# AbrahamSanders/realtime-codec-agent

Hardware: AMD Instinct MI355X
Metric: batch-encode audio-hours/hour (+ xRT and p50 frame-step latency of 1 duplex stream in `duplex`) (higher is better)
Workload: dtype f32; 1 GPU; batch MagiCodec-style encode, 16 kHz stereo, 0.1 s chunks / 2.0 s context, 256 windows per step (BASELINE configs[1]); codebook=131072x16

## Files before the change

realtime_codec_agent_amd/csrc/rca_codec.hip:

```cpp
#include <stdarg.h>

#include <algorithm>
#include <array>
#include <cmath>
#include <map>
#include <type_traits>

#include "rca_common.h"

namespace rca {
thread_local char g_err[512] = {0};
}
using namespace rca;

typedef float f32x16 __attribute__((ext_vector_type(16)));

#define RCA_LAT_MAX_FRAMES 64
#define RCA_LDS_BUDGET (152 * 1024)

typedef float f32x4 __attribute__((ext_vector_type(4)));

struct RowSrc {
    const float* base;
    int C;
    long chan_stride;
    long win_stride;
    int T;
    const long* row_off = nullptr;
    long span = 0;
    __device__ __forceinline__ long off(long b) const {
        return row_off ? row_off[b] : (b % C) * chan_stride + (b / C) * win_stride;
    }
};

__device__ __forceinline__ float lrelu(float v, float slope) { return v >= 0.0f ? v : v * slope; }

template <int KS>
__global__ __launch_bounds__(256) void conv_in_kernel(RowSrc src, const float* __restrict__ w,
                                                      const float* __restrict__ bias, float* __restrict__ y,
                                                      int B, int Cout, int Lout) {
    const long idx = (long)blockIdx.x * blockDim.x + threadIdx.x;
    if (idx >= (long)B * Lout) return;
    const int b = (int)(idx / Lout);
    const int t = (int)(idx - (long)b * Lout);
    const float* xr = src.base + src.off(b);
    constexpr int padL = KS / 2;
    float xv[KS];
#pragma unroll
    for (int kk = 0; kk < KS; ++kk) {
        const int i = t + kk - padL;
        xv[kk] = (i >= 0 && i < src.T) ? xr[i] : 0.0f;
    }
    float* yo = y + (long)b * Cout * Lout + t;
    for (int co = 0; co < Cout; ++co) {
        float acc = bias[co];
#pragma unroll
        for (int kk = 0; kk < KS; ++kk) {
            const int i = t + kk - padL;
            if (i >= 0 && i < src.T) acc = __builtin_fmaf(w[co * KS + kk], xv[kk], acc);
        }
        yo[(long)co * Lout] = acc;
    }
}

__global__ __launch_bounds__(256) void conv1d_chain_kernel(const float* __restrict__ x, const float* __restrict__ w,
                                                           const float* __restrict__ bias, float* __restrict__ y,
                                                           int B, int Cin, int Lin, int Cout, int Lout, int k, int s,
                                                           int pre, float slope, int clamp_out) {
    const long idx = (long)blockIdx.x * blockDim.x + threadIdx.x;
    if (idx >= (long)B * Cout * Lout) return;
    const int t = (int)(idx % Lout);
    const long r = idx / Lout;
    const int co = (int)(r % Cout);
    const int b = (int)(r / Cout);
    const int padL = (k - s + 1) / 2;
    const float* xb = x + (long)b * Cin * Lin;
    const float* wr = w + (long)co * Cin * k;
    float acc = bias[co];
    const int i0 = t * s - padL;
    for (int ci = 0; ci < Cin; ++ci) {
        const float* xr = xb + (long)ci * Lin;
        for (int kk = 0; kk < k; ++kk) {
            const int i = i0 + kk;
            if (i >= 0 && i < Lin) {
                float v = xr[i];
                if (pre) v = lrelu(v, slope);
                acc = __builtin_fmaf(wr[ci * k + kk], v, acc);
            }
        }
    }
    if (clamp_out) acc = acc > 1.0f ? 1.0f : (acc < -1.0f ? -1.0f : acc);
// ... 74 lines not shown
};
struct TrInfo {
    int s, padL, Lout, n_co;
};
template <int KS, int S, int TR>
struct ConvBOff {
    static constexpr int padL = (KS - S + 1) / 2;
    static constexpr int q_of(int kp, int half) {
        const int kl = 2 * kp + half, kk = kl % KS;
        const int d = TR ? -kk : kk - padL;
        return (d >= 0) ? d / S : -((-d + S - 1) / S);
    }
    static constexpr int off(int kp, int half, int U) {
        const int kl = 2 * kp + half, ci = kl / KS, kk = kl % KS;
        const int d = TR ? -kk : kk - padL;
        const int q = q_of(kp, half);
        return (ci * S + (d - q * S)) * U + 1 + q;
    }
    static constexpr int delta(int kp, int U) { return off(kp, 1, U) - off(kp, 0, U); }
    static constexpr int distinct(int k, int KPC, int U) {
        int found[4] = {0, 0, 0, 0};
        int n = 0;
        for (int kp = 0; kp < KPC; ++kp) {
            const int d = delta(kp, U);
            bool seen = false;
            for (int i = 0; i < n; ++i) seen = seen || found[i] == d;
            if (!seen && n < 4) found[n++] = d;
        }
        return found[k < n ? k : n - 1];
    }
    static constexpr int count(int KPC, int U) {
        int found[8] = {0, 0, 0, 0, 0, 0, 0, 0};
        int n = 0;
        for (int kp = 0; kp < KPC; ++kp) {
            const int d = delta(kp, U);
            bool seen = false;
            for (int i = 0; i < n; ++i) seen = seen || found[i] == d;
            if (!seen && n < 8) found[n++] = d;
        }
        return n;
    }
};

#ifndef RCA_CONV_WPB
#define RCA_CONV_WPB 1
#endif
#ifndef RCA_CONV_OCC
#define RCA_CONV_OCC 2
#endif
#ifndef RCA_CONV_PIPE
#define RCA_CONV_PIPE 1
#endif
#ifndef RCA_CONV_PRIO
#define RCA_CONV_PRIO 1
#endif
#ifndef RCA_CONV_ABUF
#define RCA_CONV_ABUF 1
#endif
#ifndef RCA_CONV_EPRIO
#define RCA_CONV_EPRIO 1
#endif
#ifdef RCA_ABL_NOBREAD
#define RCA_ABL_BREAD(x) (slope)
#else
#define RCA_ABL_BREAD(x) (x)
#endif
typedef __bf16 conv_bf16x8 __attribute__((ext_vector_type(8)));
typedef __bf16 conv_bf16x2 __attribute__((ext_vector_type(2)));
__device__ __forceinline__ unsigned conv_pack_bf16x2(float a, float b) {
    const conv_bf16x2 v = {(__bf16)a, (__bf16)b};
    return __builtin_bit_cast(unsigned, v);
}
template <int BF>
__device__ __forceinline__ void conv_split8(const float (&w)[8], uint4& hi, uint4& lo) {
    unsigned ph[4], pl[4];
#pragma unroll
    for (int j = 0; j < 4; ++j) {
        ph[j] = conv_pack_bf16x2(w[2 * j], w[2 * j + 1]);
        pl[j] = BF == 3 ? conv_pack_bf16x2(w[2 * j] - __uint_as_float(ph[j] << 16), w[2 * j + 1] - __uint_as_float(ph[j] & 0xffff0000u)) : 0u;
    }
    hi = make_uint4(ph[0], ph[1], ph[2], ph[3]);
    lo = make_uint4(pl[0], pl[1], pl[2], pl[3]);
}
template <int KS, int S, int CIC, int WM, int WN, int FUSE, int TR, int BF = 0, int FULLC = 0>
__global__ __launch_bounds__(64 * RCA_CONV_WPB, (((KS == 8 && CIC == 2) || (KS == 16 && CIC == 1)) && WM * WN < 8) ? 3 : RCA_CONV_OCC) void conv1d_mfma_kernel(const float* __restrict__ x, const float* __restrict__ wp,
                                                          const float* __restrict__ bias, float* __restrict__ y,
                                                          int Cin, int Lin, int Cout, int Lout, long Ncols, int nchunks,
                                                          int pre, float slope, FuseIn fin, TrInfo tr) {
    constexpr int MT = WM * 32;
    constexpr int NW = WN * 32;
    constexpr int U = ConvLds<S>::stride(NW);
    constexpr int KPC = CIC * KS / 2;
    constexpr int QPC = KPC / 4;
    constexpr int E = (NW + 2) * S;
    constexpr int PW = (S % 2 == 0 && !TR) ? 2 : 1;
    constexpr int RE = (E + 64 * PW - 1) / (64 * PW);
    constexpr int padL = (KS - S + 1) / 2;
    constexpr int BUF = CIC * S * U + 4;
    static_assert((CIC * KS) % 8 == 0, "chunk must hold whole weight quads");

    extern __shared__ __attribute__((aligned(16))) float xs_all[];
#ifdef RCA_CONV_TIMELINE
    long* const tl_buf = rca_prof_buf;
#endif
    RCA_TL_STAMP(tl0);

    const int lane = threadIdx.x & 63;
    const int half = lane >> 5;
    const int wave = __builtin_amdgcn_readfirstlane(threadIdx.x >> 6);
    float* xs = xs_all + wave * 2 * BUF;
    const int n_co_real = (Cout + MT - 1) / MT;
    const int n_co = TR ? n_co_real * tr.s : n_co_real;
    const long wg = blockIdx.x;
    const int xcd = (int)(wg & 7);
    const long seq = wg >> 3;
    const int co_tile_x = __builtin_amdgcn_readfirstlane((int)(seq % n_co));
    const int phase = TR ? co_tile_x / n_co_real : 0;
    const int co_tile = TR ? co_tile_x % n_co_real : co_tile_x;
    const long col_tile = (seq / n_co) * 8 + xcd;
    const long n0 = (col_tile * RCA_CONV_WPB + wave) * NW;
    const int co0 = co_tile * MT;
    if (n0 >= Ncols) return;
    const long n_base = n0 > 0 ? n0 - 1 : 0;
    const int b_base = __builtin_amdgcn_readfirstlane((int)((unsigned)n_base / (unsigned)Lout));
    const int t_base = (int)(n_base - (long)b_base * Lout);
    const int lead = n0 > 0 ? 0 : 1;
    const long left = Ncols - n_base;
    const int ncol_left = left > NW + 2 ? NW + 2 : (int)left;
    auto rel_bt = [&](int dn, int& bb, int& tt) {
        int dt = dn + t_base;
        bb = 0;
        if (Lout >= NW + 3) {
            if (dt >= Lout) { dt -= Lout; bb = 1; }
        } else {
            bb = dt / Lout;
            dt -= bb * Lout;
        }
        tt = dt;
    };

    constexpr unsigned OOB = 0x80000000u;
    const rca_rsrc_t rs_x = rca_make_rsrc(FUSE ? fin.src.base : x + (long)b_base * Cin * Lin, 0x7FFFFFFF);
    const rca_rsrc_t rs_none = rca_make_rsrc(FUSE ? fin.src.base : x, 0);
    unsigned s_boff[RE];
    int s_loff[RE];
    bool s_ok[FUSE ? RE : 1];
    float pc[FUSE ? RE : 1][6 + PW];
    rca_rsrc_t rs_pcm = rs_none;
    unsigned prow[2] = {0u, 0u};
    if (FUSE) {
        long o0, o1;
        if (fin.src.row_off) {
            const long nrows = (Ncols + Lout - 1) / Lout;
            o0 = fin.src.row_off[b_base];
            o1 = fin.src.row_off[b_base + 1 < nrows ? b_base + 1 : b_base];
        } else {
            const int C = fin.src.C;
            const int c0 = b_base % C, w0 = b_base / C;
            const int c1 = c0 + 1 == C ? 0 : c0 + 1, w1 = c0 + 1 == C ? w0 + 1 : w0;
            o0 = (long)c0 * fin.src.chan_stride + (long)w0 * fin.src.win_stride;
            o1 = (long)c1 * fin.src.chan_stride + (long)w1 * fin.src.win_stride;
        }
        const long om = o0 < o1 ? o0 : o1;
        rs_pcm = rca_make_rsrc(fin.src.base + om, 0x7FFFFFFF);
        prow[0] = (unsigned)(o0 - om);
        prow[1] = (unsigned)(o1 - om);
    }
#pragma unroll
    for (int r = 0; r < RE; ++r) {
        const int e = PW * (lane + 64 * r);
        const int slot = e / S, p = e - slot * S;
        const int dn = slot - lead;
        bool ok = e < E && dn >= 0 && dn < ncol_left;
        int bb, t;
        rel_bt(ok ? dn : 0, bb, t);
        if (TR && t >= Lin) ok = false;
        s_loff[r] = e < E ? p * U + slot : (U > NW + 2 ? U - 1 : -1);
        s_boff[r] = ok ? ((unsigned)bb * (unsigned)(Cin * Lin) + (unsigned)(t * S + p)) * 4u : OOB;
        if (FUSE) {
            s_ok[r] = ok;
            const int i = t * S + p;
            const unsigned ro = bb ? prow[1] : prow[0];
#pragma unroll
            for (int kk = 0; kk < 6 + PW; ++kk) {
                const int j = i + kk - 3;
                const unsigned off = (ok && j >= 0 && j < fin.src.T) ? (ro + (unsigned)j) * 4u : OOB;
                pc[r][kk] = rca_buffer_load_f32(rs_pcm, (int)off, 0, 0);
            }
        }
    }
    float sreg[CIC][RE][PW];
    auto stage_load = [&](int c) {
#pragma unroll
        for (int cl = 0; cl < CIC; ++cl) {
            const int ci = c * CIC + cl;
            if (FUSE) {
                const int cc = ci < Cin ? ci : 0;
                const float* wr = fin.w_in + cc * 7;
                const float bi = fin.b_in[cc];
#pragma unroll
                for (int r = 0; r < RE; ++r)
#pragma unroll
                    for (int j = 0; j < PW; ++j) {
// ... 281 lines not shown
        }
        RCA_TL_STAMP(td);
        RCA_TL_MIN(tl_load, tb, tc); RCA_TL_ADD(tl_mfma, tb, tc); RCA_TL_ADD(tl_write, tc, td);
        if (c + 1 >= nchunks) break;
        const int c2 = min(c + 2, lastc);
        stage_load(c2);
        __builtin_amdgcn_sched_barrier(0);
        __builtin_amdgcn_s_setprio(RCA_CONV_EPRIO);
        if constexpr (BF != 0) compute_b(1, c2, edge_tag);
        else if constexpr (PIPE) compute_p(1, c2, edge_tag);
        else compute_t(1, c2, edge_tag);
        __builtin_amdgcn_s_setprio(RCA_CONV_PRIO ? 3 : 2);
        __builtin_amdgcn_sched_barrier(0);
        stage_write_t(0, act_tag);
        __builtin_amdgcn_wave_barrier();
        if constexpr (PIPE) {
            read_head(0);
            __builtin_amdgcn_sched_barrier(0);
        }
    }
    };
    if (pre & 1) {
        if (edges) chunk_loop(std::true_type{}, std::true_type{});
        else chunk_loop(std::false_type{}, std::true_type{});
    } else {
        if (edges) chunk_loop(std::true_type{}, std::false_type{});
        else chunk_loop(std::false_type{}, std::false_type{});
    }

    if (RCA_CONV_EPRIO) __builtin_amdgcn_s_setprio(0);
    RCA_TL_STAMP(tl2);
    const long orow = TR ? tr.Lout : Lout;
    const bool full_rows = co0 + MT <= Cout;
    float* const yw = y + ((long)b_base * Cout + co0) * orow;
#pragma unroll
    for (int wn = 0; wn < WN; ++wn) {
        const int dn = 1 - lead + wn * 32 + (lane & 31);
        if (dn >= ncol_left) continue;
        int bb, t;
        rel_bt(dn, bb, t);
        int ocol = t;
        if (TR) {
            ocol = tr.s * t - tr.padL + phase;
            if (ocol < 0 || ocol >= (int)orow) continue;
        }
        const unsigned voff = ((unsigned)bb * (unsigned)(Cout * (int)orow) + (unsigned)ocol + (unsigned)(4 * half) * (unsigned)orow) * 4u;
        if (pre & 2) {
#pragma unroll
            for (int wm = 0; wm < WM; ++wm)
#pragma unroll
                for (int r = 0; r < 16; ++r) acc[wm][wn][r] = fmaxf(acc[wm][wn][r], acc[wm][wn][r] * slope);
        }
        if (full_rows) {
#pragma unroll
            for (int wm = 0; wm < WM; ++wm)
#pragma unroll
                for (int r = 0; r < 16; ++r) {
                    const int cu = wm * 32 + (r & 3) + 8 * (r >> 2);
                    char* const yr = reinterpret_cast<char*>(yw + (long)cu * orow);
                    *reinterpret_cast<float*>(yr + voff) = acc[wm][wn][r];
                }
        } else {
#pragma unroll
            for (int wm = 0; wm < WM; ++wm)
#pragma unroll
                for (int r = 0; r < 16; ++r) {
                    const int cu = wm * 32 + (r & 3) + 8 * (r >> 2);
                    char* const yr = reinterpret_cast<char*>(yw + (long)cu * orow);
                    if (co0 + cu + 4 * half < Cout) *reinterpret_cast<float*>(yr + voff) = acc[wm][wn][r];
                }
        }
    }
#ifdef RCA_CONV_TIMELINE
    if (tl_buf && lane == 0) {
        const long tl3 = (long)wall_clock64();
        const unsigned hw = __builtin_amdgcn_s_getreg((31 << 11) | (0 << 6) | 4);
        const unsigned xcc = __builtin_amdgcn_s_getreg((3 << 11) | (0 << 6) | 20);
        constexpr int region = KS == 4 ? 0 : KS == 8 ? 1 : KS == 10 ? 2 : KS == 16 ? 3 : KS == 3 ? 4 : 5;
        long* o = tl_buf + ((long)region * 65536 + ((blockIdx.x * RCA_CONV_WPB + wave) & 0xFFFF)) * 8;
        o[6] = tl_load | (tl_mfma << 32);
        o[7] = tl_write | ((long)nchunks << 32);
        o[0] = tl0; o[1] = tl1; o[2] = tl2; o[3] = tl3;
        o[4] = (long)hw | ((long)xcc << 32);
        o[5] = (long)KS | ((long)S << 8) | ((long)WM << 16) | ((long)wave << 24) | ((long)blockIdx.x << 32);
    }
#endif
}

template <int NWN, bool PRE>
__global__ __launch_bounds__(64, 2) void conv_first_mfma_kernel(const float* __restrict__ wp, const float* __restrict__ bias,
                                                               float* __restrict__ y, int Cout, int Lout, long Ncols, int post, float slope,
                                                               FuseIn fin) {
    constexpr int NW = NWN * 32;
    constexpr int E = (NW + 2) * 2;
    constexpr int NBLK = 2 * NWN + 1;
    constexpr int RS = 136;
    constexpr int ZERO = 128;
    constexpr int CIN = 32, KQ = CIN / 2;
    extern __shared__ __attribute__((aligned(16))) float ring[];
#ifdef RCA_CONV_TIMELINE
    long* const tl_buf = rca_prof_buf;
#endif
    RCA_TL_STAMP(tl0);
    const int lane = threadIdx.x & 63;
    const int half = lane >> 5, jl = lane & 31;
    const int n_co = Cout / 64;
    const long wg = blockIdx.x;
    const int xcd = (int)(wg & 7);
    const long seq = wg >> 3;
    const int co_tile = __builtin_amdgcn_readfirstlane((int)(seq % n_co));
    const long n0 = ((seq / n_co) * 8 + xcd) * NW;
    const int co0 = co_tile * 64;
    if (n0 >= Ncols) return;
    const long n_base = n0 > 0 ? n0 - 1 : 0;
    const int b_base = __builtin_amdgcn_readfirstlane((int)((unsigned)n_base / (unsigned)Lout));
    const int t_base = (int)(n_base - (long)b_base * Lout);
    const int lead = n0 > 0 ? 0 : 1;
    const long left = Ncols - n_base;
    const int ncol_left = left > NW + 2 ? NW + 2 : (int)left;
    auto rel_bt = [&](int dn, int& bb, int& tt) {
        int dt = dn + t_base;
        bb = dt >= Lout ? 1 : 0;
        tt = bb ? dt - Lout : dt;
    };

    const int ch_in = jl;
    float a_in[4];
#pragma unroll
    for (int m = 0; m < 4; ++m) a_in[m] = (2 * m + half < 7) ? fin.w_in[ch_in * 7 + 2 * m + half] : -0.0f;
    f32x16 b_in;
#pragma unroll
    for (int r = 0; r < 16; ++r) b_in[r] = fin.b_in[(r & 3) + 8 * (r >> 2) + 4 * half];
    long o0, o1;
    if (fin.src.row_off) {
        const long nrows = (Ncols + Lout - 1) / Lout;
        o0 = fin.src.row_off[b_base];
        o1 = fin.src.row_off[b_base + 1 < nrows ? b_base + 1 : b_base];
    } else {
        const int C = fin.src.C;
        const int c0 = b_base % C, w0 = b_base / C;
        const int c1 = c0 + 1 == C ? 0 : c0 + 1, w1 = c0 + 1 == C ? w0 + 1 : w0;
        o0 = (long)c0 * fin.src.chan_stride + (long)w0 * fin.src.win_stride;
        o1 = (long)c1 * fin.src.chan_stride + (long)w1 * fin.src.win_stride;
    }
    const long om = o0 < o1 ? o0 : o1;
    const rca_rsrc_t rs_pcm = rca_make_rsrc(fin.src.base + om, 0x7FFFFFFF);
    const unsigned prow0 = (unsigned)(o0 - om), prow1 = (unsigned)(o1 - om);
    constexpr unsigned OOB = 0x80000000u;
    auto pcm_load = [&](int bk, float (&pb)[4]) __attribute__((always_inline)) {
        const int e = 32 * bk + jl;
        const int dn = (e >> 1) - lead;
        const bool ok = e < E && dn >= 0 && dn < ncol_left;
        int bb, t;
        rel_bt(ok ? dn : 0, bb, t);
        const int i = 2 * t + (e & 1) - 3 + half;
        const unsigned ro = bb ? prow1 : prow0;
#pragma unroll
        for (int m = 0; m < 4; ++m) {
            const int j = i + 2 * m;
            const unsigned off = (ok && 2 * m + half < 7 && j >= 0 && j < fin.src.T) ? (ro + (unsigned)j) * 4u : OOB;
            pb[m] = rca_buffer_load_f32(rs_pcm, (int)off, 0, 0);
        }
    };
    auto cin_mfma = [&](int m, const float (&pb)[4], f32x16& d) __attribute__((always_inline)) {
        d = __builtin_amdgcn_mfma_f32_32x32x2f32(a_in[m], pb[m], m == 0 ? b_in : d, 0, 0, 0);
    };
    const int w_lane = 4 * half * RS + jl;
    auto cin_write = [&](int bk, f32x16& d, int r0, int r1) __attribute__((always_inline)) {
#pragma unroll
// ... 1441 lines not shown
                v.push_back(L);
                return fail(RCA_ERR_HIP, "bias pad alloc");
            }
        }
        if (pack && !tr && mfma_supported(k, s)) {
            const rca_tensor_t* t = find_tensor(ts, nt, name + ".weight");
            if ((rc = pack_weights((const float*)t->data, L)) != RCA_OK) { v.push_back(L); return rc; }
        }
        if (tr && k == 2 * s) {
            const rca_tensor_t* t = find_tensor(ts, nt, name + ".weight");
            if ((rc = pack_weights_tr((const float*)t->data, L)) != RCA_OK) { v.push_back(L); return rc; }
        }
        v.push_back(L);
        return RCA_OK;
    };
    if ((rc = add(h->enc, "enc.conv_in", 1, cfg->channels[0], cfg->k_in, 1, 0, 0, false)) != RCA_OK) return bail(rc);
    for (int i = 0; i < n; ++i) {
        const int s = cfg->strides[i];
        if ((rc = add(h->enc, "enc.down." + std::to_string(i), cfg->channels[i], cfg->channels[i + 1], 2 * s, s, 1, 0, true)) != RCA_OK)
            return bail(rc);
    }
    if ((rc = add(h->enc, "enc.conv_out", cfg->channels[n], cfg->latent_dim, cfg->k_latent, 1, 1, 0, true)) != RCA_OK) return bail(rc);
    if ((rc = add(h->dec, "dec.conv_in", cfg->codebook_dim, cfg->channels[n], cfg->k_latent, 1, 0, 0, true)) != RCA_OK) return bail(rc);
    for (int i = 0; i < n; ++i) {
        const int s = cfg->strides[n - 1 - i];
        if ((rc = add(h->dec, "dec.up." + std::to_string(i), cfg->channels[n - i], cfg->channels[n - 1 - i], 2 * s, s, 1, 1, false)) != RCA_OK)
            return bail(rc);
    }
    if ((rc = add(h->dec, "dec.conv_out", cfg->channels[0], 1, cfg->k_in, 1, 1, 0, false)) != RCA_OK) return bail(rc);

    const int J = cfg->codebook_dim, N = cfg->codebook_size, R = cfg->codebook_raw_dim, D = cfg->latent_dim;
    if ((rc = upload(ts, nt, "quantizer.in_proj.weight", (long)J * D, &h->q_in_w)) != RCA_OK) return bail(rc);
    if ((rc = upload(ts, nt, "quantizer.in_proj.bias", J, &h->q_in_b)) != RCA_OK) return bail(rc);
    float *raw = nullptr, *pw = nullptr, *pb = nullptr;
    auto free3 = [&]() { for (float* p : {raw, pw, pb}) if (p) (void)hipFree(p); };
    if ((rc = upload(ts, nt, "quantizer.codebook.weight", (long)N * R, &raw)) != RCA_OK) { free3(); return bail(rc); }
    if ((rc = upload(ts, nt, "quantizer.codebook_proj.weight", (long)J * R, &pw)) != RCA_OK) { free3(); return bail(rc); }
    if ((rc = upload(ts, nt, "quantizer.codebook_proj.bias", J, &pb)) != RCA_OK) { free3(); return bail(rc); }
    if (hipMalloc((void**)&h->cb, (size_t)N * J * 4) != hipSuccess || hipMalloc((void**)&h->hc, (size_t)N * 4) != hipSuccess ||
        hipMalloc((void**)&h->cbp, (size_t)N * J * 4) != hipSuccess || hipMalloc((void**)&h->err_flag, 4) != hipSuccess) {
        free3();
        return bail(fail(RCA_ERR_HIP, "codebook alloc"));
    }
    (void)hipMemsetAsync(h->err_flag, 0, 4, h->stream);
#ifdef RCA_CONV_TIMELINE
    if (getenv("RCA_CONV_TIMELINE_OUT")) {
        long* b = nullptr;
        (void)hipMalloc((void**)&b, (size_t)(6 << 16) * 8 * 8);
        (void)hipMemset(b, 0, (size_t)(6 << 16) * 8 * 8);
        (void)hipMemcpyToSymbol(HIP_SYMBOL(rca_prof_buf), &b, 8);
    }
#endif
    codebook_proj_kernel<<<cdiv((long)N * J, 256), 256, 0, h->stream>>>(raw, pw, pb, h->cb, N, R, J);
    codebook_norm_pack_kernel<<<cdiv(N, 256), 256, 0, h->stream>>>(h->cb, h->hc, h->cbp, N, J);
    hipError_t e = hipStreamSynchronize(h->stream);
    free3();
    if (e != hipSuccess) return bail(fail(RCA_ERR_HIP, "codebook init: %s", hipGetErrorString(e)));
    *out = h;
    return RCA_OK;
}

extern "C" int rca_codec_hop(const rca_codec_t* h, int32_t* hop) {
    if (!h || !hop) return fail(RCA_ERR_ARG, "null");
    *hop = h->hop;
    return RCA_OK;
}
extern "C" int rca_codec_num_frames(const rca_codec_t* h, int32_t T, int32_t* F) {
    if (!h || !F || T < 0) return fail(RCA_ERR_ARG, "bad argument");
    *F = (T + h->hop - 1) / h->hop;
    return RCA_OK;
}
extern "C" int rca_codec_set_variant(rca_codec_t* h, int32_t v) {
    if (!h || v < 0 || v > 2) return fail(RCA_ERR_ARG, "variant must be 0, 1 or 2");
    h->variant = v;
    return RCA_OK;
}
extern "C" int rca_codec_sync(rca_codec_t* h) {
    if (!h) return fail(RCA_ERR_ARG, "null");
    RCA_HIP(hipSetDevice(h->device));
    RCA_HIP(hipStreamSynchronize(h->stream));
    return RCA_OK;
}

template <int KS, int S, int CIC, int WM, int WN, int FUSE, int TR, int BF = 0>
static void launch_conv_cfg(const ConvLayer& L, const float* wp, int nchunks, const float* x, float* y, int Lin, int Lc, long Ncols,
                            float slope, const FuseIn& fin, const TrInfo& tr, hipStream_t st, int act) {
    constexpr int NT = RCA_CONV_WPB * WN * 32, MT = WM * 32;
    constexpr int lds = RCA_CONV_WPB * 2 * (CIC * S * ConvLds<S>::stride(WN * 32) + 4) * 4;
    static_assert(lds <= 65536, "LDS budget");
    const long col_tiles = (cdiv(Ncols, NT) + 7) / 8 * 8;
    dim3 grid((unsigned)(col_tiles * cdiv(L.cout, MT) * (TR ? tr.s : 1)));
    if constexpr (!FUSE && !TR && BF == 0) {
        if (L.cin % CIC == 0 && nchunks * CIC == L.cin) {
            conv1d_mfma_kernel<KS, S, CIC, WM, WN, 0, 0, 0, 1><<<grid, 64 * RCA_CONV_WPB, lds, st>>>(x, wp, L.bp, y, L.cin, Lin, L.cout, Lc, Ncols, nchunks, act, slope, fin, tr);
            return;
        }
    }
    conv1d_mfma_kernel<KS, S, CIC, WM, WN, FUSE, TR, BF><<<grid, 64 * RCA_CONV_WPB, lds, st>>>(x, wp, L.bp, y, L.cin, Lin, L.cout, Lc, Ncols, nchunks, act, slope, fin, tr);
}

template <int KS, int S, int CIC>
static int launch_conv_mfma(const ConvLayer& L, const float* x, float* y, int B, int Lin, int Lout, float slope, hipStream_t st,
                            const FuseIn* fuse = nullptr, int act = -1, int bf = 0) {
    if (act < 0) act = L.pre;
    const long Ncols = (long)B * Lout;
    if (bf) {
        const FuseIn none_b{};
        const TrInfo notr_b{};
        const bool big = (long)cdiv(Ncols, 64) * cdiv(L.cout, 64) >= 2048;
#define RCA_BF_LAUNCH(FU, BFM) do { \
            if (big) launch_conv_cfg<KS, S, CIC, 2, 2, FU, 0, BFM>(L, L.wp, L.nchunks, x, y, Lin, Lout, Ncols, slope, FU ? *fuse : none_b, notr_b, st, act); \
            else launch_conv_cfg<KS, S, CIC, 1, 1, FU, 0, BFM>(L, L.wp, L.nchunks, x, y, Lin, Lout, Ncols, slope, FU ? *fuse : none_b, notr_b, st, act); } while (0)
        if constexpr (KS == 4 || KS == 8 || KS == 16) {
            if (fuse) { if (bf == 3) RCA_BF_LAUNCH(1, 3); else RCA_BF_LAUNCH(1, 1); RCA_LAUNCH_CHECK(); return RCA_OK; }
        }
        if (fuse) return fail(RCA_ERR_ARG, "internal: fused first layer of this shape has no bf16 instantiation");
        if (bf == 3) RCA_BF_LAUNCH(0, 3); else RCA_BF_LAUNCH(0, 1);
#undef RCA_BF_LAUNCH
        RCA_LAUNCH_CHECK();
        return RCA_OK;
    }
    const long waves_big = (long)cdiv(Ncols, 64) * cdiv(L.cout, 64);
#ifdef RCA_CONV_FORCE_MID
    constexpr long BIG_MIN = 1L << 40, MID_MIN = 2048;
#else
    constexpr long BIG_MIN = 8192, MID_MIN = 2048;
#endif
    const FuseIn none{};
    const TrInfo notr{};
    if (fuse) {
        static const bool wide = []() { const char* e = getenv("RCA_FUSE_WIDE"); return !(e && e[0] == '0'); }();
        if constexpr (KS == 4 && S == 2) {
            const char* mi = getenv("RCA_FUSE_MFMA_IN");
            constexpr int NWN = 4;
            if (!(mi && mi[0] == '0') && wide && waves_big >= BIG_MIN && Lout >= NWN * 32 + 3 && L.cin == 32 && L.cout % 64 == 0) {
                const long col_tiles = (cdiv(Ncols, NWN * 32) + 7) / 8 * 8;
                const dim3 grid((unsigned)(col_tiles * (L.cout / 64)));
                constexpr int lds = 32 * 136 * 4;
                if (act & 1) conv_first_mfma_kernel<NWN, true><<<grid, 64, lds, st>>>(L.wp, L.bp, y, L.cout, Lout, Ncols, act & 2, slope, *fuse);
                else conv_first_mfma_kernel<NWN, false><<<grid, 64, lds, st>>>(L.wp, L.bp, y, L.cout, Lout, Ncols, act & 2, slope, *fuse);
                RCA_LAUNCH_CHECK();
                return RCA_OK;
            }
            if (wide && waves_big >= BIG_MIN && Lout >= 131 && L.cin % 2 == 0) {
                launch_conv_cfg<4, 2, 2, 2, 4, 1, 0>(L, L.wp, L.cin / 2, x, y, Lin, Lout, Ncols, slope, *fuse, notr, st, act);
                RCA_LAUNCH_CHECK();
                return RCA_OK;
            }
        }
        if (waves_big >= BIG_MIN) launch_conv_cfg<KS, S, CIC, 2, 2, 1, 0>(L, L.wp, L.nchunks, x, y, Lin, Lout, Ncols, slope, *fuse, notr, st, act);
        else launch_conv_cfg<KS, S, CIC, 1, 1, 1, 0>(L, L.wp, L.nchunks, x, y, Lin, Lout, Ncols, slope, *fuse, notr, st, act);
    } else {
        if (waves_big >= BIG_MIN) launch_conv_cfg<KS, S, CIC, 2, 2, 0, 0>(L, L.wp, L.nchunks, x, y, Lin, Lout, Ncols, slope, none, notr, st, act);
        else if (waves_big >= MID_MIN) launch_conv_cfg<KS, S, CIC, 1, 2, 0, 0>(L, L.wp, L.nchunks, x, y, Lin, Lout, Ncols, slope, none, notr, st, act);
        else if (KS == 3 && L.cout >= 64 && waves_big >= 1024) launch_conv_cfg<KS, S, CIC, (KS == 3 ? 2 : 1), 1, 0, 0>(L, L.wp, L.nchunks, x, y, Lin, Lout, Ncols, slope, none, notr, st, act);
        else launch_conv_cfg<KS, S, CIC, 1, 1, 0, 0>(L, L.wp, L.nchunks, x, y, Lin, Lout, Ncols, slope, none, notr, st, act);
    }
    RCA_LAUNCH_CHECK();
    return RCA_OK;
}

static int launch_convtr_mfma(const ConvLayer& L, const float* x, float* y, int B, int Lin, float slope, hipStream_t st) {
    const int Lc = Lin + 1;
    const long Ncols = (long)B * Lc;
    const FuseIn none{};
    const TrInfo tr{L.s, (L.k - L.s + 1) / 2, Lin * L.s, L.cout_pad / 32};
    const long waves_big = (long)cdiv(Ncols, 64) * cdiv(L.cout, 64) * L.s;
    if (L.cout > 32 && waves_big >= 2048) launch_conv_cfg<2, 1, 16, 2, 2, 0, 1>(L, L.wp_tr, L.nchunks_tr, x, y, Lin, Lc, Ncols, slope, none, tr, st, L.pre);
    else launch_conv_cfg<2, 1, 16, 1, 1, 0, 1>(L, L.wp_tr, L.nchunks_tr, x, y, Lin, Lc, Ncols, slope, none, tr, st, L.pre);
    RCA_LAUNCH_CHECK();
    return RCA_OK;
}

template <int KS, int S, int CIC, int FUSE>
static void launch_conv_ws(const ConvLayer& L, const float* x, float* y, int Lin, int Lout, long Ncols, float slope, const FuseIn& fin,
                           hipStream_t st) {
    constexpr int KPC = CIC * KS / 2, QPC = KPC / 4;
    constexpr int lds = (2 * (2 * QPC * 64 * 4) + 4 * 2 * (CIC * S * ConvLds<S>::stride(64) + 4)) * 4;
    static_assert(lds <= 160 * 1024, "LDS budget");
    auto kern = conv1d_ws_kernel<KS, S, CIC, FUSE>;
    static bool attr_done = false;
    if (!attr_done) { (void)hipFuncSetAttribute((const void*)kern, hipFuncAttributeMaxDynamicSharedMemorySize, lds); attr_done = true; }
    const long col_tiles = (cdiv(Ncols, 256) + 7) / 8 * 8;
    dim3 grid((unsigned)(col_tiles * cdiv(L.cout, 64)));
    kern<<<grid, 512, lds, st>>>(x, L.wp2, L.b, y, L.cin, Lin, L.cout, Lout, Ncols, L.nchunks2, L.pre, slope, fin);
}
static bool try_conv_ws(const ConvLayer& L, const float* x, float* y, int B, int Lin, int Lout, float slope, hipStream_t st, const FuseIn* fuse) {
    const long Ncols = (long)B * Lout;
    if (!L.wp2 || (long)cdiv(Ncols, 64) * cdiv(L.cout, 64) < 1024) return false;
    const FuseIn none{};
    if (L.k == 4 && L.s == 2) { if (fuse) launch_conv_ws<4, 2, 16, 1>(L, x, y, Lin, Lout, Ncols, slope, *fuse, st); else launch_conv_ws<4, 2, 16, 0>(L, x, y, Lin, Lout, Ncols, slope, none, st); }
    else if (L.k == 8 && L.s == 4 && !fuse) launch_conv_ws<8, 4, 8, 0>(L, x, y, Lin, Lout, Ncols, slope, none, st);
    else if (L.k == 16 && L.s == 8 && !fuse) launch_conv_ws<16, 8, 4, 0>(L, x, y, Lin, Lout, Ncols, slope, none, st);
    else if (L.k == 10 && L.s == 5 && !fuse) launch_conv_ws<10, 5, 8, 0>(L, x, y, Lin, Lout, Ncols, slope, none, st);
    else if (L.k == 3 && L.s == 1 && !fuse) launch_conv_ws<3, 1, 16, 0>(L, x, y, Lin, Lout, Ncols, slope, none, st);
    else return false;
    return true;
}

template <int K, int S, int NW>
static void launch_conv_lds(const ConvLayer& L, const float* x, long xbs, int Lvalid, float* y, int B, int Lin, int Lout, int NC, int W, int pre,
                            float slope, int clamp_out, hipStream_t st) {
    const size_t lds = ((size_t)W * (L.cin + 4) + (size_t)NW * L.cin * K) * 4;
    auto kern = conv1d_lds_kernel<K, S, NW>;
    static bool attr_done = false;
    if (!attr_done) { (void)hipFuncSetAttribute((const void*)kern, hipFuncAttributeMaxDynamicSharedMemorySize, RCA_LDS_BUDGET); attr_done = true; }
    dim3 grid(cdiv(Lout, NC), cdiv(L.cout, NW), B);
    kern<<<grid, 64 * NW, lds, st>>>(x, xbs, Lvalid, L.w, L.b, y, L.cin, Lin, L.cout, Lout, NC, W, slope, pre, clamp_out);
}
template <int S, int NW>
static void launch_convtr_lds(const ConvLayer& L, const float* x, float* y, int B, int Lin, int NC, int NTI, float slope, hipStream_t st) {
    const size_t lds = ((size_t)NTI * (L.cin + 4) + (size_t)NW * 2 * S * (L.cin + 4)) * 4;
    auto kern = convtr1d_lds_kernel<S, NW>;
    static bool attr_done = false;
    if (!attr_done) { (void)hipFuncSetAttribute((const void*)kern, hipFuncAttributeMaxDynamicSharedMemorySize, RCA_LDS_BUDGET); attr_done = true; }
    dim3 grid(cdiv((long)Lin * S, NC), cdiv(L.cout, NW), B);
    kern<<<grid, 64 * NW, lds, st>>>(x, L.w, L.w_lat, L.b, y, L.cin, Lin, L.cout, NC, NTI, slope, L.pre);
}
static bool try_conv_lds(rca_codec* h, const ConvLayer& L, const float* x, long xbs, int Lvalid, float* y, int B, int Lin, int clamp_out, hipStream_t st) {
    const float slope = h->cfg.leaky_slope;
    if (L.tr) {
        if (L.k != 2 * L.s) return false;
        const int Lout = Lin * L.s;
        const int NC = std::min(64, Lout);
        const int NTI = NC / L.s + 3;
        if (L.cin % 4 != 0) return false;
        auto fits = [&](int nw) { return ((size_t)NTI * (L.cin + 4) + (size_t)nw * L.k * (L.cin + 4)) * 4 <= RCA_LDS_BUDGET; };
#define RCA_TR(SS) if (L.s == SS) { if (fits(4)) launch_convtr_lds<SS, 4>(L, x, y, B, Lin, NC, NTI, slope, st); \
                                   else if (fits(2)) launch_convtr_lds<SS, 2>(L, x, y, B, Lin, NC, NTI, slope, st); \
                                   else if (fits(1)) launch_convtr_lds<SS, 1>(L, x, y, B, Lin, NC, NTI, slope, st); else return false; return true; }
        RCA_TR(2) RCA_TR(4) RCA_TR(5) RCA_TR(8)
#undef RCA_TR
        return false;
    }
    const int Lout = Lin / L.s;
    const int nw = L.cout >= 4 ? 4 : 1;
// ... 1067 lines not shown
```

Baseline: 3360 audio-hours/hour.

## Balance conv tail waves with mixed-tile kernel mixing big and fine tiles

Adds a mixed conv kernel where the first workgroups run large tiles and the remaining column range uses smaller tiles. A planner sizes the bulk portion from the CU count and occupancy so the final partial wave of work is split finely. This targets tail imbalance on the last dispatch round. It also lowers the threshold for choosing the 2x2 tile config when balancing is possible, which shifts some mid-sized layers onto the big tile path.

```diff
diff --git a/realtime_codec_agent_amd/csrc/rca_codec.hip b/realtime_codec_agent_amd/csrc/rca_codec.hip
--- a/realtime_codec_agent_amd/csrc/rca_codec.hip
+++ b/realtime_codec_agent_amd/csrc/rca_codec.hip
@@ -7,6 +7,7 @@
 #include <type_traits>
 
 #include "rca_common.h"
+#include "rca_conv_balance.h"
 
 namespace rca {
 thread_local char g_err[512] = {0};
@@ -247,11 +248,11 @@
     hi = make_uint4(ph[0], ph[1], ph[2], ph[3]);
     lo = make_uint4(pl[0], pl[1], pl[2], pl[3]);
 }
-template <int KS, int S, int CIC, int WM, int WN, int FUSE, int TR, int BF = 0, int FULLC = 0>
-__global__ __launch_bounds__(64 * RCA_CONV_WPB, (((KS == 8 && CIC == 2) || (KS == 16 && CIC == 1)) && WM * WN < 8) ? 3 : RCA_CONV_OCC) void conv1d_mfma_kernel(const float* __restrict__ x, const float* __restrict__ wp,
-                                                          const float* __restrict__ bias, float* __restrict__ y,
-                                                          int Cin, int Lin, int Cout, int Lout, long Ncols, int nchunks,
-                                                          int pre, float slope, FuseIn fin, TrInfo tr) {
+template <int KS, int S, int CIC, int WM, int WN, int FUSE, int TR, int BF, int FULLC>
+__device__ __forceinline__ void conv1d_mfma_body(const float* __restrict__ x, const float* __restrict__ wp,
+                                                 const float* __restrict__ bias, float* __restrict__ y,
+                                                 int Cin, int Lin, int Cout, int Lout, long Ncols, int nchunks,
+                                                 int pre, float slope, FuseIn fin, TrInfo tr, const long wg, const long n_off) {
     constexpr int MT = WM * 32;
     constexpr int NW = WN * 32;
     constexpr int U = ConvLds<S>::stride(NW);
@@ -276,14 +277,13 @@
     float* xs = xs_all + wave * 2 * BUF;
     const int n_co_real = (Cout + MT - 1) / MT;
     const int n_co = TR ? n_co_real * tr.s : n_co_real;
-    const long wg = blockIdx.x;
     const int xcd = (int)(wg & 7);
     const long seq = wg >> 3;
     const int co_tile_x = __builtin_amdgcn_readfirstlane((int)(seq % n_co));
     const int phase = TR ? co_tile_x / n_co_real : 0;
     const int co_tile = TR ? co_tile_x % n_co_real : co_tile_x;
     const long col_tile = (seq / n_co) * 8 + xcd;
-    const long n0 = (col_tile * RCA_CONV_WPB + wave) * NW;
+    const long n0 = n_off + (col_tile * RCA_CONV_WPB + wave) * NW;
     const int co0 = co_tile * MT;
     if (n0 >= Ncols) return;
     const long n_base = n0 > 0 ? n0 - 1 : 0;
@@ -731,9 +731,28 @@
         o[7] = tl_write | ((long)nchunks << 32);
         o[0] = tl0; o[1] = tl1; o[2] = tl2; o[3] = tl3;
         o[4] = (long)hw | ((long)xcc << 32);
-        o[5] = (long)KS | ((long)S << 8) | ((long)WM << 16) | ((long)wave << 24) | ((long)blockIdx.x << 32);
+        o[5] = (long)KS | ((long)S << 8) | ((long)(WM | (WN << 4)) << 16) | ((long)wave << 24) | ((long)blockIdx.x << 32);
     }
 #endif
+}
+
+template <int KS, int S, int CIC, int WM, int WN, int FUSE, int TR, int BF = 0, int FULLC = 0>
+__global__ __launch_bounds__(64 * RCA_CONV_WPB, (((KS == 8 && CIC == 2) || (KS == 16 && CIC == 1)) && WM * WN < 8) ? 3 : RCA_CONV_OCC) void conv1d_mfma_kernel(const float* __restrict__ x, const float* __restrict__ wp,
+                                                          const float* __restrict__ bias, float* __restrict__ y,
+                                                          int Cin, int Lin, int Cout, int Lout, long Ncols, int nchunks,
+                                                          int pre, float slope, FuseIn fin, TrInfo tr) {
+    conv1d_mfma_body<KS, S, CIC, WM, WN, FUSE, TR, BF, FULLC>(x, wp, bias, y, Cin, Lin, Cout, Lout, Ncols, nchunks, pre, slope, fin, tr, blockIdx.x, 0);
+}
+
+template <int KS, int S, int CIC, int WM, int WN, int WM2, int WN2, int FULLC>
+__global__ __launch_bounds__(64 * RCA_CONV_WPB, (((KS == 8 && CIC == 2) || (KS == 16 && CIC == 1)) && WM * WN < 8) ? 3 : RCA_CONV_OCC) void conv1d_mfma_mixed_kernel(const float* __restrict__ x, const float* __restrict__ wp,
+                                                          const float* __restrict__ bias, float* __restrict__ y,
+                                                          int Cin, int Lin, int Cout, int Lout, long Ncols, int nchunks,
+                                                          int pre, float slope, unsigned n_bulk_wg, long fine_col0) {
+    const FuseIn fin{};
+    const TrInfo tr{};
+    if (blockIdx.x < n_bulk_wg) conv1d_mfma_body<KS, S, CIC, WM, WN, 0, 0, 0, FULLC>(x, wp, bias, y, Cin, Lin, Cout, Lout, Ncols, nchunks, pre, slope, fin, tr, blockIdx.x, 0);
+    else conv1d_mfma_body<KS, S, CIC, WM2, WN2, 0, 0, 0, FULLC>(x, wp, bias, y, Cin, Lin, Cout, Lout, Ncols, nchunks, pre, slope, fin, tr, blockIdx.x - n_bulk_wg, fine_col0);
 }
 
 template <int NWN, bool PRE>
@@ -2341,6 +2360,43 @@
     return RCA_OK;
 }
 
+template <int KS, int S, int CIC, int WM, int WN>
+static bool launch_conv_balanced(const ConvLayer& L, const float* wp, int nchunks, const float* x, float* y, int Lin, int Lc, long Ncols,
+                                 float slope, hipStream_t st, int act, int lds) {
+    constexpr int NT = RCA_CONV_WPB * WN * 32, MT = WM * 32;
+    const char* on = getenv("RCA_CONV_BALANCE");
+    if (on && on[0] == '0') return false;
+    const long total = cdiv(Ncols, NT);
+    const int n_co = (int)cdiv(L.cout, MT);
+    ConvBalancePlan p;
+    if (!conv_balance_parse(getenv("RCA_CONV_BALANCE_PLAN"), total, WM, WN, &p)) {
+        static int simds_of[64], occ_of[64];
+        int dev = 0;
+        if (hipGetDevice(&dev) != hipSuccess || dev < 0 || dev >= 64) return false;
+        if (!simds_of[dev]) {
+            int cus = 0, blocks = 0;
+            if (hipDeviceGetAttribute(&cus, hipDeviceAttributeMultiprocessorCount, dev) != hipSuccess || cus <= 0) return false;
+            if (hipOccupancyMaxActiveBlocksPerMultiprocessor(&blocks, conv1d_mfma_kernel<KS, S, CIC, WM, WN, 0, 0, 0, 1>, 64 * RCA_CONV_WPB, lds) != hipSuccess || blocks < 4)
+                return false;
+            occ_of[dev] = blocks * RCA_CONV_WPB / 4;
+            simds_of[dev] = 4 * cus;
+        }
+        p = conv_balance_plan(total, n_co, simds_of[dev], occ_of[dev], WM, WN);
+    }
+    if (!p.fine_wn) return false;
+    const long fine_col0 = p.bulk_col_tiles * NT;
+    const long n_bulk_wg = p.bulk_col_tiles * n_co;
+    const long fine_tiles = (cdiv(Ncols - fine_col0, RCA_CONV_WPB * p.fine_wn * 32) + 7) / 8 * 8;
+    const long n_wg = n_bulk_wg + fine_tiles * cdiv(L.cout, p.fine_wm * 32);
+    if (n_wg >= (1L << 31)) return false;
+    const dim3 grid((unsigned)n_wg);
+    if (WM * WN == 4 && p.fine_wn == 2)
+        conv1d_mfma_mixed_kernel<KS, S, CIC, WM, WN, 1, (WM * WN == 4 ? 2 : 1), 1><<<grid, 64 * RCA_CONV_WPB, lds, st>>>(x, wp, L.bp, y, L.cin, Lin, L.cout, Lc, Ncols, nchunks, act, slope, (unsigned)n_bulk_wg, fine_col0);
+    else
+        conv1d_mfma_mixed_kernel<KS, S, CIC, WM, WN, 1, 1, 1><<<grid, 64 * RCA_CONV_WPB, lds, st>>>(x, wp, L.bp, y, L.cin, Lin, L.cout, Lc, Ncols, nchunks, act, slope, (unsigned)n_bulk_wg, fine_col0);
+    return true;
+}
+
 template <int KS, int S, int CIC, int WM, int WN, int FUSE, int TR, int BF = 0>
 static void launch_conv_cfg(const ConvLayer& L, const float* wp, int nchunks, const float* x, float* y, int Lin, int Lc, long Ncols,
                             float slope, const FuseIn& fin, const TrInfo& tr, hipStream_t st, int act) {
@@ -2351,6 +2407,9 @@
     dim3 grid((unsigned)(col_tiles * cdiv(L.cout, MT) * (TR ? tr.s : 1)));
     if constexpr (!FUSE && !TR && BF == 0) {
         if (L.cin % CIC == 0 && nchunks * CIC == L.cin) {
+            if constexpr (KS >= 8 && WN == 2 && WM <= 2) {
+                if (launch_conv_balanced<KS, S, CIC, WM, WN>(L, wp, nchunks, x, y, Lin, Lc, Ncols, slope, st, act, lds)) return;
+            }
             conv1d_mfma_kernel<KS, S, CIC, WM, WN, 0, 0, 0, 1><<<grid, 64 * RCA_CONV_WPB, lds, st>>>(x, wp, L.bp, y, L.cin, Lin, L.cout, Lc, Ncols, nchunks, act, slope, fin, tr);
             return;
         }
@@ -2381,10 +2440,18 @@
     }
     const long waves_big = (long)cdiv(Ncols, 64) * cdiv(L.cout, 64);
 #ifdef RCA_CONV_FORCE_MID
-    constexpr long BIG_MIN = 1L << 40, MID_MIN = 2048;
+    constexpr long BIG_MIN = 1L << 40, MID_MIN = 2048, BIG_BAL_MIN = 1L << 40;
 #else
     constexpr long BIG_MIN = 8192, MID_MIN = 2048;
+#ifdef RCA_CONV_BIG_BAL_MIN
+    constexpr long BIG_BAL_MIN = RCA_CONV_BIG_BAL_MIN;
+#else
+    constexpr long BIG_BAL_MIN = 3072;
 #endif
+#endif
+    const char* bal = getenv("RCA_CONV_BALANCE");
+    const bool balanced = KS >= 8 && !fuse && !(bal && bal[0] == '0') && L.cin % CIC == 0 && L.nchunks * CIC == L.cin;
+    const long big_min = balanced && BIG_BAL_MIN < BIG_MIN ? BIG_BAL_MIN : BIG_MIN;
     const FuseIn none{};
     const TrInfo notr{};
     if (fuse) {
@@ -2410,7 +2477,7 @@
         if (waves_big >= BIG_MIN) launch_conv_cfg<KS, S, CIC, 2, 2, 1, 0>(L, L.wp, L.nchunks, x, y, Lin, Lout, Ncols, slope, *fuse, notr, st, act);
         else launch_conv_cfg<KS, S, CIC, 1, 1, 1, 0>(L, L.wp, L.nchunks, x, y, Lin, Lout, Ncols, slope, *fuse, notr, st, act);
     } else {
-        if (waves_big >= BIG_MIN) launch_conv_cfg<KS, S, CIC, 2, 2, 0, 0>(L, L.wp, L.nchunks, x, y, Lin, Lout, Ncols, slope, none, notr, st, act);
+        if (waves_big >= big_min) launch_conv_cfg<KS, S, CIC, 2, 2, 0, 0>(L, L.wp, L.nchunks, x, y, Lin, Lout, Ncols, slope, none, notr, st, act);
         else if (waves_big >= MID_MIN) launch_conv_cfg<KS, S, CIC, 1, 2, 0, 0>(L, L.wp, L.nchunks, x, y, Lin, Lout, Ncols, slope, none, notr, st, act);
         else if (KS == 3 && L.cout >= 64 && waves_big >= 1024) launch_conv_cfg<KS, S, CIC, (KS == 3 ? 2 : 1), 1, 0, 0>(L, L.wp, L.nchunks, x, y, Lin, Lout, Ncols, slope, none, notr, st, act);
         else launch_conv_cfg<KS, S, CIC, 1, 1, 0, 0>(L, L.wp, L.nchunks, x, y, Lin, Lout, Ncols, slope, none, notr, st, act);
diff --git a/realtime_codec_agent_amd/csrc/rca_conv_balance.h b/realtime_codec_agent_amd/csrc/rca_conv_balance.h
--- /dev/null
+++ b/realtime_codec_agent_amd/csrc/rca_conv_balance.h
@@ -0,0 +1,56 @@
+#pragma once
+
+struct ConvBalancePlan {
+    long bulk_col_tiles;
+    int fine_wm, fine_wn;
+    long finish;
+    long finish_single;
+};
+
+static inline long conv_balance_cdiv(long a, long b) { return (a + b - 1) / b; }
+
+static inline long conv_balance_finish(long total, long bulk, int n_co_bulk, int simds, int wm, int wn, int fwm, int fwn) {
+    const long bulk_waves = bulk * n_co_bulk;
+    const long fine_waves = (total - bulk) * (wn / fwn) * n_co_bulk * (wm / fwm);
+    return conv_balance_cdiv(bulk_waves, simds) * (wm * wn) + conv_balance_cdiv(fine_waves, simds) * (fwm * fwn);
+}
+
+static inline ConvBalancePlan conv_balance_plan(long total_col_tiles, int n_co_bulk, int simds, int occ_bulk, int wm, int wn) {
+    ConvBalancePlan p{total_col_tiles, 0, 0, 0, 0};
+    if (total_col_tiles <= 0 || n_co_bulk <= 0 || simds <= 0 || occ_bulk <= 0) return p;
+    const long waves = total_col_tiles * n_co_bulk, round = (long)simds * occ_bulk;
+    p.finish = p.finish_single = conv_balance_cdiv(waves, simds) * (wm * wn);
+    if (waves < round) return p;
+    const long rounds = waves / round;
+    static const int fine[2][2] = {{1, 2}, {1, 1}};
+    for (long r = rounds; r >= 1 && r + 1 >= rounds; --r) {
+        long bulk = (r * round / n_co_bulk) / 8 * 8;
+        if (bulk > total_col_tiles) bulk = total_col_tiles / 8 * 8;
+        if (bulk <= 0 || bulk >= total_col_tiles) continue;
+        for (const auto& f : fine) {
+            if (f[0] > wm || f[1] > wn || f[0] * f[1] >= wm * wn) continue;
+            const long fin = conv_balance_finish(total_col_tiles, bulk, n_co_bulk, simds, wm, wn, f[0], f[1]);
+            if (fin < p.finish) p = ConvBalancePlan{bulk, f[0], f[1], fin, p.finish_single};
+        }
+    }
+    return p;
+}
+
+static inline bool conv_balance_parse(const char* s, long total_col_tiles, int wm, int wn, ConvBalancePlan* out) {
+    if (!s || !*s) return false;
+    long bulk = 0;
+    const char* c = s;
+    if (*c < '0' || *c > '9') return false;
+    for (; *c >= '0' && *c <= '9'; ++c) bulk = bulk < (1L << 40) ? bulk * 10 + (*c - '0') : bulk;
+    if (*c++ != ':') return false;
+    int fwn = 0;
+    if (c[0] == '3' && c[1] == '2' && c[2] == 'x' && c[3] == '6' && c[4] == '4' && !c[5]) fwn = 2;
+    else if (c[0] == '3' && c[1] == '2' && c[2] == 'x' && c[3] == '3' && c[4] == '2' && !c[5]) fwn = 1;
+    else return false;
+    if (fwn > wn || 1 * fwn >= wm * wn) return false;
+    if (bulk > total_col_tiles) bulk = total_col_tiles;
+    bulk = bulk / 8 * 8;
+    if (bulk >= total_col_tiles) *out = ConvBalancePlan{total_col_tiles, 0, 0, 0, 0};
+    else *out = ConvBalancePlan{bulk, 1, fwn, 0, 0};
+    return true;
+}
```

Measured after the change: 3451 audio-hours/hour (median of 6 runs). 2.7% higher.
